# FKGSOFTWARE/TERRA-GAN

Measured on AMD Instinct MI355X. Metric: DSM tiles/sec train-step (G+D) at 256x256 bs=16, higher is better.
Workload: dtype f32; 1 GPU; BASELINE configs[1]: 256x256 1-ch DSM tiles, batch 16 per GPU, fp32, PConv-UNet G + PatchGAN D + L1/VGG-perceptual/TV/boundary(0.5) losses + 2x Adam; global_batch=16, tile=256, parallelism=single-gpu, launch=eager, vgg_weights=deterministic stand-in (ImageNet weights not fetchable offline; same FLOPs), vgg_trunk=forward Winograd F(2x2,3x3), dgrads F(4x4,3x3) (DESIGN 2b)

## Files before the change

### include/terragan_hip.h

```cpp
#ifndef TERRAGAN_HIP_H
#define TERRAGAN_HIP_H

#include <stddef.h>
#include <stdint.h>

#ifdef __cplusplus
extern "C" {
#endif

typedef void* tg_stream_t;

enum { TG_OK = 0, TG_ERR_ARG = -1, TG_ERR_LAUNCH = -2, TG_ERR_WS = -3 };
enum { TG_ACT_NONE = 0, TG_ACT_RELU = 1, TG_ACT_LEAKY = 2 };
enum { TG_PREC_F32 = 0, TG_PREC_BF16 = 1, TG_PREC_F32_WINO4 = 2 };

typedef struct TgConv {
    int32_t B, H, W, Cin;
    int32_t Ho, Wo, Cout;
    int32_t k, stride, pad;
    int32_t precision;
} TgConv;

int tg_version(void);
const char* tg_last_error(void);
// ... 20 lines not shown
int tg_conv_fwd_p(const TgConv* g, const float* x, const float* in_mask, const float* w, const float* wprep,
                  const float* bias, const float* ratio, int act, float slope, float* y, float* ws,
                  size_t ws_bytes, tg_stream_t stream);
int tg_conv_fwd_pool(const TgConv* g, const float* x, const float* in_mask, const float* w, const float* wprep,
                     const float* bias, const float* ratio, int act, float slope, float* y, float* pool_y, float* ws,
                     size_t ws_bytes, tg_stream_t stream);
int tg_conv_pool_code_supported(const TgConv* g);
int tg_conv_fwd_pool_code(const TgConv* g, const float* x, const float* w, const float* wprep, const float* bias,
                          float* pool_y, unsigned char* code, float* ws, size_t ws_bytes, tg_stream_t stream);
int tg_maxpool2_bwd_code(const float* dout, const unsigned char* code, int B, int Ho, int Wo, int C, float* dx,
                         tg_stream_t stream);
typedef struct TgSparseMap {
    const uint32_t* bits;
    const int32_t* list;
    const int32_t* count;
    const uint64_t* pix;
    int32_t nb, tiles_y, tiles_x, _pad;
} TgSparseMap;
size_t tg_vgg_sparse_map_bytes(int nb, int H, int W, const char* plan);
int tg_vgg_sparse_map(const float* x, const float* mask, int nb, int H, int W, const char* plan, void* buf, size_t buf_bytes,
                      int* ticket, TgSparseMap* maps, tg_stream_t stream);
int tg_conv_dgrad_sparse(const TgConv* g, const float* dy, const float* w, const float* wprep, const float* x_act, int act,
                         float slope, const uint32_t* gate_bits, float* dx, const TgSparseMap* sp, float* ws, size_t ws_bytes,
                         tg_stream_t stream);
int tg_conv_dgrad_sparse_planned(const TgConv* g, int gate, const TgSparseMap* sp);
int tg_maxpool2_bwd_code_sparse(const float* dout, const unsigned char* code, int B, int Ho, int Wo, int C, float* dx,
                                const TgSparseMap* sp, tg_stream_t stream);
int tg_conv_fwd_sparse(const TgConv* g, const float* x, const float* w, const float* wprep, const float* bias, int act,
                       float slope, float* y, float* pool_y, unsigned char* code, const TgSparseMap* sp, float* ws,
                       size_t ws_bytes, tg_stream_t stream);
typedef struct TgBnAct {
    const float *mean, *rstd, *gamma, *beta;
    int32_t act;
    float slope;
} TgBnAct;
int tg_conv_bnin_supported(const TgConv* g, int wgrad);
int tg_conv_fwd_bnin(const TgConv* g, const float* x, const TgBnAct* bn, const float* w, const float* bias, int act,
                     float slope, float* y, float* ws, size_t ws_bytes, tg_stream_t stream);
int tg_conv_wgrad_bnin(const TgConv* g, const float* x, const TgBnAct* bn, const float* dy, float* dw, float* db, float* ws,
                       size_t ws_bytes, tg_stream_t stream);
int tg_conv_dgrad_p(const TgConv* g, const float* dy, const float* w, const float* wprep, const float* in_mask,
                    const float* x_act, int act, float slope, float* dx, int accumulate, float* ws,
                    size_t ws_bytes, tg_stream_t stream);
int tg_relu_gate_pack(const float* a, int64_t rows, int C, uint32_t* bits, tg_stream_t stream);
int tg_conv_dgrad_gbits(const TgConv* g, const float* dy, const float* w, const float* wprep, const float* in_mask,
                        const uint32_t* gate_bits, float* dx, int accumulate, float* ws, size_t ws_bytes, tg_stream_t stream);

int tg_set_cu_reserve(int cus);
int tg_set_work_stealing(int mode);

size_t tg_conv_wgrad_ws_bytes(const TgConv* g);
int tg_conv_wgrad(const TgConv* g, const float* x, const float* in_mask, const float* dy,
                  float* dw, float* db, float* ws, size_t ws_bytes, tg_stream_t stream);

int tg_fold_cin(const float* w3, int cout, int taps, int cin, float* w1, tg_stream_t stream);


int tg_mask_update(const float* mask, int B, int H, int W, int k, int stride, int pad, int Ho,
                   int Wo, float* mask_out, float* ratio, tg_stream_t stream);
int tg_mask_up_merge(const float* up_mask, const float* skip_mask, int B, int h, int w, int H,
                     int W, float* out, tg_stream_t stream);

#define TG_MASK_PYRAMID_MAX 24
typedef struct TgMaskOp {
    int kind, H, W, Ho, Wo, k, stride, pad;
    const float* in;
    const float* in2;
    float* out;
    float* out2;
} TgMaskOp;
typedef struct TgMaskPyramid {
    int nops, _pad;
    TgMaskOp op[TG_MASK_PYRAMID_MAX];
} TgMaskPyramid;
int tg_mask_pyramid(const TgMaskPyramid* pm, int B, tg_stream_t stream);


size_t tg_bn_ws_bytes(int64_t rows, int C);
int tg_bn_stats(const float* y, int64_t rows, int C, float eps, float momentum, float* save_mean,
                float* save_rstd, float* running_mean, float* running_var,
                int64_t* num_batches_tracked, float* ws, size_t ws_bytes, tg_stream_t stream);
int tg_bn_fwd(const float* y, int64_t rows, int C, float eps, float momentum, const float* gamma,
              const float* beta, int act, float slope, float* save_mean, float* save_rstd,
              float* running_mean, float* running_var, int64_t* num_batches_tracked, float* out,
              float* ws, size_t ws_bytes, tg_stream_t stream);
int tg_bn_eval_stats(const float* running_mean, const float* running_var, int C, float eps,
                     float* mean, float* rstd, tg_stream_t stream);
int tg_bn_act_fwd(const float* y, int64_t rows, int C, const float* mean, const float* rstd,
                  const float* gamma, const float* beta, int act, float slope, float* out,
                  tg_stream_t stream);
int tg_bn_act_bwd(const float* dout, const float* y, int64_t rows, int C, const float* mean,
                  const float* rstd, const float* gamma, const float* beta, int act, float slope,
                  const float* ratio, float* dy, float* dgamma, float* dbeta, float* dbias, float* ws,
                  size_t ws_bytes, tg_stream_t stream);
int tg_bn_bwd_conv1_supported(int64_t rows, int C);
size_t tg_bn_conv1_ws_bytes(int64_t rows, int C);
int tg_bn_act_bwd_conv1(const float* dz, const float* w, int B, int H, int W, const float* y, int C, const float* mean,
                        const float* rstd, const float* gamma, const float* beta, int act, float slope, const float* ratio,
                        float* dy, float* dgamma, float* dbeta, float* dbias, float* ws, size_t ws_bytes, tg_stream_t stream);
int tg_act_bwd(const float* dout, const float* out, int64_t rows, int C, int act, float slope,
               const float* ratio, float* din, tg_stream_t stream);


int tg_upcat_fwd(const float* up, const float* skip, const float* out_mask, int B, int h, int w,
                 int Cu, int H, int W, int Cs, float* out, tg_stream_t stream);
int tg_upcat_bn_supported(int B, int h, int w, int Cu, int H, int W, int Cs);
// ... 308 lines not shown
```

### terra-gan_amd/csrc/pointwise.hip

```cpp
#include <math.h>
#include <string.h>

#include "common.h"

static thread_local char g_err[512] = "";
void tg_set_error(const char* fmt, ...) {
    va_list ap;
    va_start(ap, fmt);
    vsnprintf(g_err, sizeof(g_err), fmt, ap);
    va_end(ap);
}
extern "C" const char* tg_last_error(void) { return g_err; }
extern "C" int tg_version(void) { return 100; }

static size_t align_up(size_t v, size_t a) { return (v + a - 1) / a * a; }
static inline hipStream_t S(tg_stream_t s) { return (hipStream_t)s; }

constexpr int CR_MAXPASS = 4;

struct ColGeom {
    int cpp;
    int rlanes;
    int npass;
    int grid;
// ... 300 lines not shown
    TG_REQUIRE(pm && B > 0 && pm->nops >= 1 && pm->nops <= TG_MASK_PYRAMID_MAX, "tg_mask_pyramid: bad arguments");
    for (int i = 0; i < pm->nops; ++i) {
        const TgMaskOp& op = pm->op[i];
        TG_REQUIRE(op.in && op.out && (op.kind == 0 ? op.out2 != nullptr : op.in2 != nullptr), "tg_mask_pyramid: op %d: null pointer", i);
        TG_REQUIRE(op.H > 0 && op.W > 0 && op.Ho > 0 && op.Wo > 0, "tg_mask_pyramid: op %d: bad dims", i);
        if (op.kind == 0)
            TG_REQUIRE(op.k > 0 && op.stride > 0 && op.pad >= 0 && op.Ho == (op.H + 2 * op.pad - op.k) / op.stride + 1 &&
                       op.Wo == (op.W + 2 * op.pad - op.k) / op.stride + 1, "tg_mask_pyramid: op %d: Ho/Wo inconsistent", i);
    }
    hipLaunchKernelGGL(mask_pyramid_kernel, dim3(B), dim3(1024), 0, S(stream), *pm);
    TG_CHECK_LAUNCH("mask_pyramid_kernel");
    return TG_OK;
}

constexpr int VSM_MAX_OPS = 24, VSM_MAX_CONV = 16, VSM_LDS_WORDS = 4096;
struct VggMapArgs {
    const uint32_t* x;
    const float* mask;
    int nb, H, W, nops, nconv;
    char ops[VSM_MAX_OPS];
    int tiles_y[VSM_MAX_CONV], tiles_x[VSM_MAX_CONV];
    int32_t* count[VSM_MAX_CONV];
    uint32_t* bits[VSM_MAX_CONV];
    int32_t* list[VSM_MAX_CONV];
    unsigned char* flags[VSM_MAX_CONV];
    uint64_t* d0;
    int rows_per_slice;
    int* ticket;
};
__device__ __forceinline__ uint32_t vsm_even_bits(uint64_t v) {
    v &= 0x5555555555555555ull;
    v = (v | (v >> 1)) & 0x3333333333333333ull;
    v = (v | (v >> 2)) & 0x0f0f0f0f0f0f0f0full;
    v = (v | (v >> 4)) & 0x00ff00ff00ff00ffull;
    v = (v | (v >> 8)) & 0x0000ffff0000ffffull;
    v = (v | (v >> 16)) & 0x00000000ffffffffull;
    return (uint32_t)v;
}
__device__ __forceinline__ uint64_t vsm_row_mask(int W, int w, int WW) {
    return (w == WW - 1 && (W & 63)) ? (1ull << (W & 63)) - 1 : ~0ull;
}
__device__ __forceinline__ bool vsm_last_arrival(int* ctr, int n, int* s_last) {
    __builtin_amdgcn_s_waitcnt(0);
    __syncthreads();
    if (threadIdx.x == 0) {
        __threadfence();
        const bool last = atomicAdd(ctr, 1) == n - 1;
        if (last) __threadfence();
        *s_last = last;
    }
    __syncthreads();
    return *s_last;
}
__global__ __launch_bounds__(1024) void vgg_sparse_map_kernel(const VggMapArgs a) {
    extern __shared__ uint64_t vsm[];
    __shared__ int scan[1024];
    __shared__ int s_last;
    const int tid = threadIdx.x, lane = tid & 63, wave = tid >> 6, b = blockIdx.y;
    int H = a.H, W = a.W, WW = (W + 63) >> 6;
    uint64_t* cur = vsm;
    uint64_t* nxt = vsm + H * WW;
    uint64_t* d0 = a.d0 + (size_t)b * H * WW;
    {
        const uint32_t* xp = a.x + (size_t)b * H * W;
        const uint32_t* tp = a.x + ((size_t)a.nb + b) * H * W;
        const float* mp = a.mask ? a.mask + (size_t)b * H * W : nullptr;
        const int ubeg = blockIdx.x * a.rows_per_slice * WW, uend = min(H, (blockIdx.x + 1) * a.rows_per_slice) * WW;
        for (int u0 = ubeg + wave; u0 < uend; u0 += 16 * 8) {
            uint32_t pv[8], tv[8];
            float mv[8];
#pragma unroll
            for (int k = 0; k < 8; ++k) {
                const int u = u0 + 16 * k, y = u / WW, px = (u - y * WW) * 64 + lane;
                pv[k] = tv[k] = 0;
                mv[k] = 1.f;
                if (u < uend && px < W) {
                    pv[k] = xp[(size_t)y * W + px]; tv[k] = tp[(size_t)y * W + px];
                    if (mp) mv[k] = mp[(size_t)y * W + px];
                }
            }
#pragma unroll
            for (int k = 0; k < 8; ++k) {
                const uint64_t m = __ballot(pv[k] != tv[k] || mv[k] != 1.f);
                if (lane == 0 && u0 + 16 * k < uend) d0[u0 + 16 * k] = m;
            }
        }
    }
    if (!vsm_last_arrival(a.ticket + b, (int)gridDim.x, &s_last)) return;
    for (int u = tid; u < H * WW; u += 1024) cur[u] = d0[u];
    if (tid == 0) __hip_atomic_store(a.ticket + b, 0, __ATOMIC_RELAXED, __HIP_MEMORY_SCOPE_AGENT);
    __syncthreads();
    int ci = 0;
    for (int o = 0; o < a.nops; ++o) {
        if (a.ops[o] == 'C') {
            for (int u = tid; u < H * WW; u += 1024) {
                const int y = u / WW, w = u - y * WW;
                uint64_t r = 0;
                for (int dy = -1; dy <= 1; ++dy) {
                    const int yy = y + dy;
                    if (yy < 0 || yy >= H) continue;
                    const uint64_t* row = cur + yy * WW;
                    const uint64_t v = row[w];
                    r |= v | (v << 1) | (v >> 1);
                    if (w > 0) r |= row[w - 1] >> 63;
                    if (w + 1 < WW) r |= row[w + 1] << 63;
                }
                nxt[u] = r & vsm_row_mask(W, w, WW);
            }
            __syncthreads();
            uint64_t* t = cur; cur = nxt; nxt = t;
            const int ty_n = a.tiles_y[ci], tx_n = a.tiles_x[ci], tiles = ty_n * tx_n;
            for (int t2 = tid; t2 < tiles; t2 += 1024) {
                const int ty = t2 / tx_n, tx = t2 - ty * tx_n;
                const int w = (16 * tx) >> 6, sh = (16 * tx) & 63;
                uint64_t any = 0;
                for (int y = 16 * ty; y < min(16 * ty + 16, H); ++y) any |= (cur[y * WW + w] >> sh) & 0xffffull;
                a.flags[ci][(size_t)b * tiles + t2] = any ? 1 : 0;
            }
            ++ci;
        } else {
            const int H2 = H >> 1, W2 = W >> 1, WW2 = (W2 + 63) >> 6;
            for (int u = tid; u < H2 * WW2; u += 1024) {
                const int y = u / WW2, w = u - y * WW2;
                const uint64_t* r0 = cur + (2 * y) * WW;
                const uint64_t* r1 = r0 + WW;
                const uint64_t s0 = r0[2 * w] | r1[2 * w];
                const uint64_t s1 = 2 * w + 1 < WW ? r0[2 * w + 1] | r1[2 * w + 1] : 0;
                const uint64_t v = (uint64_t)vsm_even_bits(s0 | (s0 >> 1)) | ((uint64_t)vsm_even_bits(s1 | (s1 >> 1)) << 32);
                nxt[u] = v & vsm_row_mask(W2, w, WW2);
            }
            H = H2; W = W2; WW = WW2;
            __syncthreads();
            uint64_t* t = cur; cur = nxt; nxt = t;
        }
        __syncthreads();
    }
    if (!vsm_last_arrival(a.ticket + a.nb, a.nb, &s_last)) return;
    for (int c = 0; c < a.nconv; ++c) {
        const int n = a.nb * a.tiles_y[c] * a.tiles_x[c], nw = (n + 31) >> 5;
        int carry = 0;
        for (int w0 = 0; w0 < nw; w0 += 1024) {
            const int w = w0 + tid;
            uint32_t word = 0;
            if (w < nw) {
                const uint4* fp = reinterpret_cast<const uint4*>(a.flags[c] + 32 * (size_t)w);
                const uint4 f0 = fp[0], f1 = fp[1];
                const uint32_t fw[8] = {f0.x, f0.y, f0.z, f0.w, f1.x, f1.y, f1.z, f1.w};
#pragma unroll
                for (int i = 0; i < 8; ++i)
#pragma unroll
                    for (int j = 0; j < 4; ++j) word |= ((fw[i] >> (8 * j)) & 1u) << (4 * i + j);
                if (32 * w + 32 > n) word &= (1u << (n - 32 * w)) - 1u;
                a.bits[c][w] = word;
            }
            const int pc = __popc(word);
            scan[tid] = pc;
            __syncthreads();
            for (int d = 1; d < 1024; d <<= 1) {
                const int v = tid >= d ? scan[tid - d] : 0;
                __syncthreads();
                scan[tid] += v;
                __syncthreads();
            }
            int pos = carry + scan[tid] - pc;
            for (uint32_t m = word; m; m &= m - 1) a.list[c][pos++] = 32 * w + __ffs(m) - 1;
            carry += scan[1023];
            __syncthreads();
        }
        if (tid == 0) *a.count[c] = carry;
    }
    if (tid == 0) __hip_atomic_store(a.ticket + a.nb, 0, __ATOMIC_RELAXED, __HIP_MEMORY_SCOPE_AGENT);
}

struct VsmLayout {
    int nconv, nops, H, W;
    size_t d0;
    int tiles_y[VSM_MAX_CONV], tiles_x[VSM_MAX_CONV];
    size_t count[VSM_MAX_CONV], bits[VSM_MAX_CONV], list[VSM_MAX_CONV], flags[VSM_MAX_CONV];
    size_t bytes;
};
static bool vsm_layout(int nb, int H, int W, const char* plan, VsmLayout& L) {
    if (nb <= 0 || H <= 0 || W <= 0 || !plan) return false;
    if ((size_t)H * ((W + 63) / 64) > VSM_LDS_WORDS) return false;
    L = VsmLayout{};
    L.H = H; L.W = W;
    L.d0 = 0;
    size_t off = align_up((size_t)nb * H * ((W + 63) / 64) * sizeof(uint64_t), 16);
    int h = H, w = W;
    for (const char* c = plan; *c; ++c) {
        if (L.nops == VSM_MAX_OPS) return false;
        ++L.nops;
        if (*c == 'M') {
            h >>= 1; w >>= 1;
            if (h <= 0 || w <= 0) return false;
        } else if (*c == 'C') {
            if (L.nconv == VSM_MAX_CONV) return false;
            const int i = L.nconv++;
            L.tiles_y[i] = cdiv(h, 16); L.tiles_x[i] = cdiv(w, 16);
            const size_t n = (size_t)nb * L.tiles_y[i] * L.tiles_x[i];
            if (n > ((size_t)1 << 30)) return false;
            L.count[i] = off; off += 16;
            L.bits[i] = off; off += align_up((n + 31) / 32, 4) * 4;
            L.list[i] = off; off += align_up(n, 4) * 4;
            L.flags[i] = off; off += align_up(n, 32);
        } else {
            return false;
        }
    }
    L.bytes = off;
    return L.nconv > 0;
}
extern "C" size_t tg_vgg_sparse_map_bytes(int nb, int H, int W, const char* plan) {
    VsmLayout L;
    return vsm_layout(nb, H, W, plan, L) ? L.bytes : 0;
}
extern "C" int tg_vgg_sparse_map(const float* x, const float* mask, int nb, int H, int W, const char* plan, void* buf, size_t buf_bytes,
                                 int* ticket, TgSparseMap* maps, tg_stream_t stream) {
    VsmLayout L;
    TG_REQUIRE(x && buf && ticket && maps, "tg_vgg_sparse_map: null pointer");
    TG_REQUIRE(vsm_layout(nb, H, W, plan, L), "tg_vgg_sparse_map: geometry not supported (tg_vgg_sparse_map_bytes is 0)");
    TG_REQUIRE(buf_bytes >= L.bytes && (reinterpret_cast<uintptr_t>(buf) & 15) == 0, "tg_vgg_sparse_map: buffer too small or unaligned");
    VggMapArgs a = {};
    a.x = reinterpret_cast<const uint32_t*>(x);
    a.mask = mask;
    a.nb = nb; a.H = H; a.W = W; a.nops = L.nops; a.nconv = L.nconv; a.ticket = ticket;
    for (int i = 0; i < L.nops; ++i) a.ops[i] = plan[i];
    char* base = static_cast<char*>(buf);
    a.d0 = reinterpret_cast<uint64_t*>(base + L.d0);
    const int slices = cdiv(H, 8) < cdiv(256, nb) ? cdiv(H, 8) : cdiv(256, nb);
    a.rows_per_slice = cdiv(H, slices);
    for (int i = 0; i < L.nconv; ++i) {
        a.tiles_y[i] = L.tiles_y[i]; a.tiles_x[i] = L.tiles_x[i];
        a.count[i] = reinterpret_cast<int32_t*>(base + L.count[i]);
        a.bits[i] = reinterpret_cast<uint32_t*>(base + L.bits[i]);
        a.list[i] = reinterpret_cast<int32_t*>(base + L.list[i]);
        a.flags[i] = reinterpret_cast<unsigned char*>(base + L.flags[i]);
        maps[i] = TgSparseMap{a.bits[i], a.list[i], a.count[i], mask ? a.d0 : nullptr, nb, L.tiles_y[i], L.tiles_x[i], 0};
    }
    const size_t lds = 2 * (size_t)H * ((W + 63) / 64) * sizeof(uint64_t);
    static bool opted[64] = {};
    int dev = 0;
    (void)hipGetDevice(&dev);
    if (dev < 0 || dev >= 64 || !opted[dev]) {
        if (hipFuncSetAttribute(reinterpret_cast<const void*>(vgg_sparse_map_kernel), hipFuncAttributeMaxDynamicSharedMemorySize,
                                (int)(2 * VSM_LDS_WORDS * sizeof(uint64_t))) != hipSuccess) {
            tg_set_error("tg_vgg_sparse_map: LDS opt-in failed");
            return TG_ERR_LAUNCH;
        }
        if (dev >= 0 && dev < 64) opted[dev] = true;
    }
    hipLaunchKernelGGL(vgg_sparse_map_kernel, dim3(cdiv(H, a.rows_per_slice), nb), dim3(1024), lds, S(stream), a);
    TG_CHECK_LAUNCH("vgg_sparse_map_kernel");
    return TG_OK;
}

struct BnStatF {
    const float* y;
    int C;
    __device__ BnStatF group(int g, int64_t rows_g) const { return BnStatF{y + (size_t)g * rows_g * C, C}; }
    __device__ void operator()(int64_t r, int c, float (&q)[2]) const {
        float d = y[r * C + c] - y[c];
        q[0] += d;
        q[1] += d * d;
    }
    __device__ void quad(int64_t r, int c0, float (&q)[2][4]) const {
        const f32x4 v = *reinterpret_cast<const f32x4*>(y + r * C + c0);
        const f32x4 sh = *reinterpret_cast<const f32x4*>(y + c0);
#pragma unroll
        for (int e = 0; e < 4; ++e) {
            float d = v[e] - sh[e];
            q[0][e] += d;
            q[1][e] += d * d;
        }
    }
};
__global__ __launch_bounds__(256) void bn_finalize_kernel(const float* __restrict__ partial, int nblocks, int C,
                                                          const float* __restrict__ y, int64_t rows, float eps,
                                                          float momentum, float* __restrict__ mean_out,
                                                          float* __restrict__ rstd_out, float* __restrict__ rm,
                                                          float* __restrict__ rv, int64_t* __restrict__ nbt) {
    if (blockIdx.x == 0 && threadIdx.x == 0 && nbt) *nbt += 1;
    double q[2];
    int c;
    if (!final_reduce<2>(partial, nblocks, C, q, &c)) return;
    const double n = (double)rows;
    const double md = q[0] / n;
    double var = q[1] / n - md * md;
    if (var < 0.0) var = 0.0;
    const double mean = (double)y[c] + md;
    mean_out[c] = (float)mean;
    rstd_out[c] = (float)(1.0 / sqrt(var + (double)eps));
    if (rm) rm[c] = (float)((1.0 - (double)momentum) * (double)rm[c] + (double)momentum * mean);
    if (rv) rv[c] = (float)((1.0 - (double)momentum) * (double)rv[c] + (double)momentum * var * (n / (n - 1.0)));
}
extern "C" size_t tg_bn_ws_bytes(int64_t rows, int C) {
    if (rows <= 0 || C <= 0) return 0;
    ColGeom g = col_geom(rows, C);
    int grid = g.grid;
    if (C % 4 == 0) {
        ColGeom4 g4 = col_geom4(rows, C);
        if (g4.grid > grid) grid = g4.grid;
    }
    return align_up((size_t)grid * 5 * C, 64) * sizeof(float);
}
// ... 1858 lines not shown
```

### terra-gan_amd/csrc/wino.inc

```
#pragma once
#include <utility>

struct WinoGeom {
    int tiles_x, tiles_y, total_work, chunks_per_split, nt;
    int sy_min, sx_min;
    int interleave;
    int* qctr;
    const uint32_t* sp_bits;
    const int* sp_list;
    const int* sp_count;
    int sp_tiles, sp_nb;
};
struct WinoWeights {
    long sn, sk, stap;
    int kyu[3], kxv[3];
    int k_fast;
};
typedef unsigned int u32x4 __attribute__((ext_vector_type(4)));
constexpr int WINO_BN = 64;
constexpr int WINO_V = 16 * 64 * 8;
constexpr int WINO_U = 16 * WINO_BN * 8;
constexpr int WINO_PPIX = 18 * 18;
constexpr int WINO_P = WINO_PPIX * 8;
constexpr int WINO_LDS_FLOATS = 2 * WINO_V + 2 * WINO_U + WINO_P;
// ... 1074 lines not shown
#pragma unroll
    for (int i = 0; i < 8; ++i)
#pragma unroll
        for (int r = 0; r < 16; ++r) {
            const int row = 32 * mw + (r & 3) + 8 * (r >> 2) + 4 * (lane >> 5);
            slab[(size_t)i * 4096 + row * 64 + 32 * nw + (lane & 31)] = acc[i][r];
        }
}

__global__ __launch_bounds__(256) void wino_wgrad_reduce_kernel(const float* __restrict__ slabs, float* __restrict__ dw, int Cout,
                                                                int Cin, int ntco, int ntci, int splits) {
    const int total = Cout * Cin;
    for (int idx = blockIdx.x * 256 + threadIdx.x; idx < total; idx += gridDim.x * 256) {
        const int col = idx & 63, row = (idx >> 6) & 63, tile = idx >> 12;
        const int tco = tile % ntco, tci = tile / ntco;
        float u[16];
#pragma unroll
        for (int i = 0; i < 16; ++i) u[i] = 0.f;
        const size_t sstride = (size_t)ntci * ntco * 16 * 4096;
        const float* sl = slabs + ((size_t)tile * 16) * 4096 + row * 64 + col;
        int sp = 0;
        for (; sp + 4 <= splits; sp += 4) {
            float v[4][16];
#pragma unroll
            for (int k = 0; k < 4; ++k)
#pragma unroll
                for (int i = 0; i < 16; ++i) v[k][i] = sl[(size_t)(sp + k) * sstride + (size_t)i * 4096];
#pragma unroll
            for (int k = 0; k < 4; ++k)
#pragma unroll
                for (int i = 0; i < 16; ++i) u[i] += v[k][i];
        }
        for (; sp < splits; ++sp)
#pragma unroll
            for (int i = 0; i < 16; ++i) u[i] += sl[(size_t)sp * sstride + (size_t)i * 4096];
        float t[3][4];
#pragma unroll
        for (int b = 0; b < 4; ++b) {
            t[0][b] = u[0 * 4 + b] + 0.5f * (u[1 * 4 + b] + u[2 * 4 + b]);
            t[1][b] = 0.5f * (u[1 * 4 + b] - u[2 * 4 + b]);
            t[2][b] = 0.5f * (u[1 * 4 + b] + u[2 * 4 + b]) + u[3 * 4 + b];
        }
        const int co = tco * 64 + 4 * (row & 15) + (row >> 4), ci = tci * 64 + 4 * (col & 15) + (col >> 4);
        float* o = dw + ((size_t)co * 9) * Cin + ci;
#pragma unroll
        for (int uu = 0; uu < 3; ++uu) {
            o[(size_t)(uu * 3 + 0) * Cin] = t[uu][0] + 0.5f * (t[uu][1] + t[uu][2]);
            o[(size_t)(uu * 3 + 1) * Cin] = 0.5f * (t[uu][1] - t[uu][2]);
            o[(size_t)(uu * 3 + 2) * Cin] = 0.5f * (t[uu][1] + t[uu][2]) + t[uu][3];
        }
    }
}

static bool wino_wgrad_ok(const TgConv* g, const float* in_mask) {
    static const bool off = getenv("TG_NO_WINO") != nullptr || getenv("TG_NO_WINO_WGRAD") != nullptr;
    if (off || in_mask != nullptr) return false;
    if (g->precision == TG_PREC_BF16 && g->Cin > 256) return false;
    if (g->k != 3 || g->stride != 1 || (g->Cin % 64) != 0 || (g->Cout % 64) != 0 || g->Ho < 16 || g->Wo < 16) return false;
    if ((size_t)g->B * g->H * g->W * g->Cin * 4 >= ((size_t)1 << 31) || (size_t)g->B * g->Ho * g->Wo * g->Cout * 4 >= ((size_t)1 << 31))
        return false;
    return true;
}
static WinoWgradGeom wino_wgrad_plan(const TgConv* g) {
    WinoWgradGeom q = {};
    q.strips_x = cdiv(g->Wo, 16);
    q.tiles_y = cdiv(g->Ho, 2);
    q.nstrips = g->B * q.tiles_y * q.strips_x;
    q.ntco = g->Cout / 64;
    q.ntci = g->Cin / 64;
    const int tiles = q.ntco * q.ntci;
    int smax = q.nstrips / 8 < 512 ? q.nstrips / 8 : 512;
    if (smax < 1) smax = 1;
    const int splits = choose_splits_k(tiles, smax, WINO_PLAN_CUS, q.nstrips, 0.03);
    q.steps_per_split = cdiv(q.nstrips, splits);
    q.splits = cdiv(q.nstrips, q.steps_per_split);
    return q;
}
static size_t wino_wgrad_ws_floats(const TgConv* g) {
    if (!wino_wgrad_ok(g, nullptr)) return 0;
    const WinoWgradGeom q = wino_wgrad_plan(g);
    return (size_t)q.splits * q.ntco * q.ntci * 16 * 4096;
}
static int launch_wino_wgrad(const TgConv* g, const WgradParams& p, float* dw, float* ws, hipStream_t s) {
    const WinoWgradGeom q = wino_wgrad_plan(g);
    const size_t lds = (size_t)WINO_WG_LDS_FLOATS * sizeof(float);
    static LdsOptIn opt;
    if (int rc = lds_opt_in(opt, reinterpret_cast<const void*>(wino_wgrad_kernel), lds, "wino wgrad")) return rc;
    {
        const double by = 4.0 * ((double)p.B * p.H * p.W * p.C + (double)p.Mpix * p.Cout + (double)p.Cout * p.Ktot);
        ProfScope ps(s, 1, 2.0 * p.Mpix * (double)p.Cout * p.Ktot * g_alg_scale, by, p.Cout, p.Ktot, p.Mpix, p.C, q.splits, 4164);
        ps.r.route = WR_WGRAD;
        hipLaunchKernelGGL(wino_wgrad_kernel, dim3(q.ntco * q.ntci * q.splits), dim3(WINO_THREADS), lds, s, p, q, ws);
    }
    TG_CHECK_LAUNCH("wino_wgrad_kernel");
    hipLaunchKernelGGL(wino_wgrad_reduce_kernel, dim3(ew_grid((int64_t)g->Cout * g->Cin, 256)), dim3(256), 0, s, ws, dw, g->Cout,
                       g->Cin, q.ntco, q.ntci, q.splits);
    TG_CHECK_LAUNCH("wino_wgrad_reduce_kernel");
    return TG_OK;
}
```

### terra-gan_amd/csrc/wino16.inc

```
#pragma once

constexpr int W16_IMG = 16 * 64 * 16;
constexpr int W16_P = WINO_PPIX * 16;
constexpr size_t W16_LDS_BYTES = 4 * (size_t)W16_IMG * 2 + (size_t)W16_P * 4;
constexpr int W16_PP = WINO_PPIX * 24;
constexpr size_t W16_PIPE_LDS_BYTES = 4 * (size_t)W16_IMG * 2 + (size_t)W16_PP * 4;

__host__ __device__ __forceinline__ int w16_pos(int row, int c) { return ((((c >> 3) ^ (row >> 4)) & 1) << 3) + (c & 7); }

__device__ void wino_weights16_body(const float* __restrict__ w, __bf16* __restrict__ U, int N, int K, const WinoWeights& ww) {
    const int NT = N / WINO_BN, K2 = K >> 1;
    const size_t total = (size_t)N * K2;
    for (size_t idx = (size_t)blockIdx.x * 256 + threadIdx.x; idx < total; idx += (size_t)gridDim.x * 256) {
        int n, k2;
        if (ww.k_fast) { k2 = (int)(idx % K2); n = (int)(idx / K2); }
        else { n = (int)(idx % N); k2 = (int)(idx / N); }
        float u[2][16];
#pragma unroll
        for (int h = 0; h < 2; ++h) {
            const float* wp = w + (size_t)n * ww.sn + (size_t)(2 * k2 + h) * ww.sk;
            float g[3][3];
#pragma unroll
            for (int a = 0; a < 3; ++a)
#pragma unroll
// ... 709 lines not shown
            }
        }
    }
    float* slab = slabs + ((size_t)work * 16 + 8 * xh) * 4096;
#pragma unroll
    for (int i = 0; i < 8; ++i)
#pragma unroll
        for (int r = 0; r < 16; ++r) {
            const int row = 32 * mw + (r & 3) + 8 * (r >> 2) + 4 * (lane >> 5);
            slab[(size_t)i * 4096 + row * 64 + 32 * nw + (lane & 31)] = acc[i][r];
        }
}

static bool wino16_wgrad_ok(const TgConv* g, const float* in_mask) {
    static const bool off = getenv("TG_NO_WINO") != nullptr || getenv("TG_NO_WINO_WGRAD") != nullptr || getenv("TG_NO_WINO16") != nullptr ||
                            getenv("TG_NO_WINO16_WGRAD") != nullptr;
    if (off || in_mask != nullptr || g->precision != TG_PREC_BF16) return false;
    if (g->k != 3 || g->stride != 1 || (g->Cin % 64) != 0 || (g->Cout % 64) != 0 || g->Ho < 16 || g->Wo < 32) return false;
    if ((size_t)g->B * g->H * g->W * g->Cin * 4 >= ((size_t)1 << 31) || (size_t)g->B * g->Ho * g->Wo * g->Cout * 4 >= ((size_t)1 << 31))
        return false;
    return true;
}
static WinoWgradGeom wino16_wgrad_plan(const TgConv* g) {
    WinoWgradGeom q = {};
    q.strips_x = cdiv(g->Wo, 32);
    q.tiles_y = cdiv(g->Ho, 2);
    q.nstrips = g->B * q.tiles_y * q.strips_x;
    q.ntco = g->Cout / 64;
    q.ntci = g->Cin / 64;
    const int tiles = q.ntco * q.ntci;
    int smax = q.nstrips / 4 < 512 ? q.nstrips / 4 : 512;
    if (smax < 1) smax = 1;
    const int splits = choose_splits_k(tiles, smax, WINO_PLAN_CUS, q.nstrips, 0.03);
    q.steps_per_split = cdiv(q.nstrips, splits);
    q.splits = cdiv(q.nstrips, q.steps_per_split);
    return q;
}
static size_t wino16_wgrad_ws_floats(const TgConv* g) {
    if (!wino16_wgrad_ok(g, nullptr)) return 0;
    const WinoWgradGeom q = wino16_wgrad_plan(g);
    return (size_t)q.splits * q.ntco * q.ntci * 16 * 4096;
}
static int launch_wino16_wgrad(const TgConv* g, const WgradParams& p, float* dw, float* ws, hipStream_t s) {
    const WinoWgradGeom q = wino16_wgrad_plan(g);
    static LdsOptIn opt;
    if (int rc = lds_opt_in(opt, reinterpret_cast<const void*>(wino16_wgrad_kernel), W16G_LDS_BYTES, "wino16 wgrad")) return rc;
    {
        const double by = 4.0 * ((double)p.B * p.H * p.W * p.C + (double)p.Mpix * p.Cout + (double)p.Cout * p.Ktot);
        ProfScope ps(s, 3, 2.0 * p.Mpix * (double)p.Cout * p.Ktot * g_alg_scale, by, p.Cout, p.Ktot, p.Mpix, p.C, q.splits, 4116);
        ps.r.route = WR_WGRAD;
        hipLaunchKernelGGL(wino16_wgrad_kernel, dim3(q.ntco * q.ntci * q.splits), dim3(WINO_THREADS), W16G_LDS_BYTES, s, p, q, ws);
    }
    TG_CHECK_LAUNCH("wino16_wgrad_kernel");
    hipLaunchKernelGGL(wino_wgrad_reduce_kernel, dim3(ew_grid((int64_t)g->Cout * g->Cin, 256)), dim3(256), 0, s, ws, dw, g->Cout,
                       g->Cin, q.ntco, q.ntci, q.splits);
    TG_CHECK_LAUNCH("wino_wgrad_reduce_kernel");
    return TG_OK;
}
```

### terra-gan_amd/tg_hip/lib.py

```python
import ctypes as C
import os

import torch

_HERE = os.path.dirname(os.path.abspath(__file__))
LIB_PATH = os.environ.get("TG_HIP_LIB") or os.path.join(os.path.dirname(_HERE), "lib", "libterragan_hip.so")


class TgConv(C.Structure):
    _fields_ = [(n, C.c_int32) for n in ("B", "H", "W", "Cin", "Ho", "Wo", "Cout", "k", "stride", "pad", "precision")]


TG_MASK_PYRAMID_MAX = 24


class TgMaskOp(C.Structure):
    _fields_ = [(n, C.c_int32) for n in ("kind", "H", "W", "Ho", "Wo", "k", "stride", "pad")] + \
               [(n, C.c_void_p) for n in ("in_", "in2", "out", "out2")]


class TgMaskPyramid(C.Structure):
    _fields_ = [("nops", C.c_int32), ("_pad", C.c_int32), ("op", TgMaskOp * TG_MASK_PYRAMID_MAX)]


# ... 7 lines not shown

class TgRasterPlan(C.Structure):
    _fields_ = [(n, C.c_int32) for n in ("H", "W", "wh", "ww", "overlap", "ny", "nx")]


TG_EVAL_MAX_CLASSES = 8


class TgAreaClasses(C.Structure):
    _fields_ = [("n_edges", C.c_int32), ("_pad", C.c_int32), ("px", C.c_int64 * (TG_EVAL_MAX_CLASSES - 1))]


TG_EDT_FAR, TG_EDT_MAX_SIDE, TG_DEPTH_MAX_CLASSES = 0x7fffffff, 32767, 8


class TgDepthClasses(C.Structure):
    _fields_ = [("n_edges", C.c_int32), ("_pad", C.c_int32), ("d2", C.c_int32 * (TG_DEPTH_MAX_CLASSES - 1))]


TG_FLOW_OUT, TG_FLOW_UNDECIDED, TG_FLOW_PIT, TG_FLOW_FAR, TG_FLOW_MAX_ROUNDS = 9, 254, 255, 0x7fffffff, 32
TG_FLOW_BASIN_COUNTS, TG_FLOW_COMPARE_COUNTS = 3, 19
TG_STREAM_HEAD, TG_STREAM_INTERIOR, TG_STREAM_JUNCTION, TG_STREAM_ORDER_BINS = 1, 2, 3, 15
TG_STREAM_ORDER_COUNTS = 1 + 2 * TG_STREAM_ORDER_BINS
TG_FLOOD_MAX_STAGES = 8
TG_FLOOD_COUNTS = 6 + 3 * TG_FLOOD_MAX_STAGES
TG_MFD_MAX_EXPONENT, TG_MFD_COUNTS = 8, 5
TG_TEX_OCTAVES, TG_TEX_SCALES, TG_TEX_NSUM = 5, 10, 3
TG_VGM_OCTAVES, TG_VGM_SCALES = 6, 12
TG_VGM_POWER, TG_VGM_EXPONENTIAL, TG_VGM_SPHERICAL = 0, 1, 2


class TgFloodStages(C.Structure):
    _fields_ = [("s", C.c_float * TG_FLOOD_MAX_STAGES)]


class TgError(RuntimeError):
    pass


P, I, I64, F, SZ, D = C.c_void_p, C.c_int, C.c_int64, C.c_float, C.c_size_t, C.c_double
CP = C.POINTER(TgConv)
RP = C.POINTER(TgRasterPlan)

SIGNATURES = {
    "tg_version": (I, []),
    "tg_last_error": (C.c_char_p, []),
    "tg_conv_fwd_ws_bytes": (SZ, [CP]),
    "tg_conv_fwd": (I, [CP, P, P, P, P, P, I, F, P, P, SZ, P]),
    "tg_conv_dgrad_ws_bytes": (SZ, [CP]),
    "tg_conv_dgrad": (I, [CP, P, P, P, P, I, P, SZ, P]),
    "tg_conv_dgrad_gated": (I, [CP, P, P, P, P, I, F, P, P, SZ, P]),
    "tg_set_cu_reserve": (I, [I]),
    "tg_set_work_stealing": (I, [I]),
    "tg_conv_wprep_bytes": (SZ, [CP, I]),
    "tg_conv_wprep": (I, [CP, I, P, P, P]),
    "tg_conv_wprep_item_bytes": (SZ, []),
    "tg_conv_wprep_item": (I, [CP, I, P, P, P]),
    "tg_conv_wprep_run": (I, [P, I, P]),
    "tg_conv_fwd_p": (I, [CP, P, P, P, P, P, P, I, F, P, P, SZ, P]),
    "tg_conv_fwd_pool": (I, [CP, P, P, P, P, P, P, I, F, P, P, P, SZ, P]),
    "tg_conv_pool_code_supported": (I, [CP]),
    "tg_conv_fwd_pool_code": (I, [CP, P, P, P, P, P, P, P, SZ, P]),
    "tg_maxpool2_bwd_code": (I, [P, P, I, I, I, I, P, P]),
    "tg_vgg_sparse_map_bytes": (SZ, [I, I, I, C.c_char_p]),
    "tg_vgg_sparse_map": (I, [P, P, I, I, I, C.c_char_p, P, SZ, P, C.POINTER(TgSparseMap), P]),
    "tg_conv_dgrad_sparse": (I, [CP, P, P, P, P, I, F, P, P, C.POINTER(TgSparseMap), P, SZ, P]),
    "tg_conv_dgrad_sparse_planned": (I, [CP, I, C.POINTER(TgSparseMap)]),
    "tg_maxpool2_bwd_code_sparse": (I, [P, P, I, I, I, I, P, C.POINTER(TgSparseMap), P]),
    "tg_conv_fwd_sparse": (I, [CP, P, P, P, P, I, F, P, P, P, C.POINTER(TgSparseMap), P, SZ, P]),
    "tg_conv_bnin_supported": (I, [CP, I]),
    "tg_conv_fwd_bnin": (I, [CP, P, C.POINTER(TgBnAct), P, P, I, F, P, P, SZ, P]),
    "tg_conv_wgrad_bnin": (I, [CP, P, C.POINTER(TgBnAct), P, P, P, P, SZ, P]),
    "tg_conv_dgrad_p": (I, [CP, P, P, P, P, P, I, F, P, I, P, SZ, P]),
    "tg_relu_gate_pack": (I, [P, I64, I, P, P]),
    "tg_conv_dgrad_gbits": (I, [CP, P, P, P, P, P, P, I, P, SZ, P]),
    "tg_conv_wgrad_ws_bytes": (SZ, [CP]),
    "tg_conv_wgrad": (I, [CP, P, P, P, P, P, P, SZ, P]),
    "tg_fold_cin": (I, [P, I, I, I, P, P]),
    "tg_mask_update": (I, [P, I, I, I, I, I, I, I, I, P, P, P]),
    "tg_mask_up_merge": (I, [P, P, I, I, I, I, I, P, P]),
    "tg_mask_pyramid": (I, [C.POINTER(TgMaskPyramid), I, P]),
    "tg_bn_ws_bytes": (SZ, [I64, I]),
    "tg_bn_stats": (I, [P, I64, I, F, F, P, P, P, P, P, P, SZ, P]),
    "tg_bn_eval_stats": (I, [P, P, I, F, P, P, P]),
    "tg_bn_act_fwd": (I, [P, I64, I, P, P, P, P, I, F, P, P]),
    "tg_bn_fwd": (I, [P, I64, I, F, F, P, P, I, F, P, P, P, P, P, P, P, SZ, P]),
    "tg_bn_act_bwd": (I, [P, P, I64, I, P, P, P, P, I, F, P, P, P, P, P, P, SZ, P]),
    "tg_bn_bwd_conv1_supported": (I, [I64, I]),
    "tg_bn_conv1_ws_bytes": (SZ, [I64, I]),
    "tg_bn_act_bwd_conv1": (I, [P, P, I, I, I, P, I, P, P, P, P, I, F, P, P, P, P, P, P, SZ, P]),
    "tg_act_bwd": (I, [P, P, I64, I, I, F, P, P, P]),
    "tg_upcat_fwd": (I, [P, P, P, I, I, I, I, I, I, I, P, P]),
    "tg_upcat_bn_supported": (I, [I, I, I, I, I, I, I]),
    "tg_upcat_fwd_bn": (I, [P, C.POINTER(TgBnAct), P, P, I, I, I, I, I, I, I, P, P]),
    "tg_upcat_bwd": (I, [P, I, I, I, I, I, I, I, P, P, P]),
    "tg_sigmoid_composite_fwd": (I, [P, P, P, I64, P, P]),
    "tg_sigmoid_composite_bwd": (I, [P, P, P, I64, P, P, P]),
    "tg_maxpool2_fwd": (I, [P, I, I, I, I, P, P]),
    "tg_maxpool2_bwd": (I, [P, P, I, I, I, I, I, P, P]),
    "tg_pixel_loss_ws_bytes": (SZ, [I, I, I]),
    "tg_pixel_losses": (I, [P, P, P, P, I, I, I, F, F, F, F, P, P, P, I, P, SZ, P]),
    "tg_reduce_ws_bytes": (SZ, [I64]),
    "tg_l1_mean": (I, [P, P, I64, F, P, P, P, P, SZ, P]),
    "tg_l1_mean_relu": (I, [P, P, I64, F, P, P, P, P, SZ, P]),
    "tg_bce_logits": (I, [P, I64, F, F, P, P, P, P, SZ, P]),
    "tg_adam": (I, [P, P, P, P, I64, D, D, D, D, I, F, P]),
# ... 125 lines not shown
```

Measured before the change: 1088 tiles/s.

## Split VGG sparse-map kernel into staged launches and widen Winograd wgrad reduce

```diff
diff --git a/include/terragan_hip.h b/include/terragan_hip.h
--- a/include/terragan_hip.h
+++ b/include/terragan_hip.h
@@ -96,6 +96,7 @@
 size_t tg_conv_wgrad_ws_bytes(const TgConv* g);
 int tg_conv_wgrad(const TgConv* g, const float* x, const float* in_mask, const float* dy,
                   float* dw, float* db, float* ws, size_t ws_bytes, tg_stream_t stream);
+int64_t tg_wgrad_reduce_wide_launches(void);
 
 int tg_fold_cin(const float* w3, int cout, int taps, int cin, float* w1, tg_stream_t stream);
 
diff --git a/terra-gan_amd/csrc/pointwise.hip b/terra-gan_amd/csrc/pointwise.hip
--- a/terra-gan_amd/csrc/pointwise.hip
+++ b/terra-gan_amd/csrc/pointwise.hip
@@ -376,6 +376,7 @@
     __syncthreads();
     return *s_last;
 }
+template <int STAGE>
 __global__ __launch_bounds__(1024) void vgg_sparse_map_kernel(const VggMapArgs a) {
     extern __shared__ uint64_t vsm[];
     __shared__ int scan[1024];
@@ -385,7 +386,7 @@
     uint64_t* cur = vsm;
     uint64_t* nxt = vsm + H * WW;
     uint64_t* d0 = a.d0 + (size_t)b * H * WW;
-    {
+    if constexpr (STAGE == 0 || STAGE == 1) {
         const uint32_t* xp = a.x + (size_t)b * H * W;
         const uint32_t* tp = a.x + ((size_t)a.nb + b) * H * W;
         const float* mp = a.mask ? a.mask + (size_t)b * H * W : nullptr;
@@ -410,57 +411,64 @@
             }
         }
     }
-    if (!vsm_last_arrival(a.ticket + b, (int)gridDim.x, &s_last)) return;
-    for (int u = tid; u < H * WW; u += 1024) cur[u] = d0[u];
-    if (tid == 0) __hip_atomic_store(a.ticket + b, 0, __ATOMIC_RELAXED, __HIP_MEMORY_SCOPE_AGENT);
-    __syncthreads();
-    int ci = 0;
-    for (int o = 0; o < a.nops; ++o) {
-        if (a.ops[o] == 'C') {
-            for (int u = tid; u < H * WW; u += 1024) {
-                const int y = u / WW, w = u - y * WW;
-                uint64_t r = 0;
-                for (int dy = -1; dy <= 1; ++dy) {
-                    const int yy = y + dy;
-                    if (yy < 0 || yy >= H) continue;
-                    const uint64_t* row = cur + yy * WW;
-                    const uint64_t v = row[w];
-                    r |= v | (v << 1) | (v >> 1);
-                    if (w > 0) r |= row[w - 1] >> 63;
-                    if (w + 1 < WW) r |= row[w + 1] << 63;
+    if constexpr (STAGE == 1) return;
+    if constexpr (STAGE == 0)
+        if (!vsm_last_arrival(a.ticket + b, (int)gridDim.x, &s_last)) return;
+    if constexpr (STAGE == 0 || STAGE == 2) {
+        for (int u = tid; u < H * WW; u += 1024) cur[u] = d0[u];
+        if constexpr (STAGE == 0)
+            if (tid == 0) __hip_atomic_store(a.ticket + b, 0, __ATOMIC_RELAXED, __HIP_MEMORY_SCOPE_AGENT);
+        __syncthreads();
+        int ci = 0;
+        for (int o = 0; o < a.nops; ++o) {
+            if (a.ops[o] == 'C') {
+                for (int u = tid; u < H * WW; u += 1024) {
+                    const int y = u / WW, w = u - y * WW;
+                    uint64_t r = 0;
+                    for (int dy = -1; dy <= 1; ++dy) {
+                        const int yy = y + dy;
+                        if (yy < 0 || yy >= H) continue;
+                        const uint64_t* row = cur + yy * WW;
+                        const uint64_t v = row[w];
+                        r |= v | (v << 1) | (v >> 1);
+                        if (w > 0) r |= row[w - 1] >> 63;
+                        if (w + 1 < WW) r |= row[w + 1] << 63;
+                    }
+                    nxt[u] = r & vsm_row_mask(W, w, WW);
                 }
-                nxt[u] = r & vsm_row_mask(W, w, WW);
+                __syncthreads();
+                uint64_t* t = cur; cur = nxt; nxt = t;
+                const int ty_n = a.tiles_y[ci], tx_n = a.tiles_x[ci], tiles = ty_n * tx_n;
+                for (int t2 = tid; t2 < tiles; t2 += 1024) {
+                    const int ty = t2 / tx_n, tx = t2 - ty * tx_n;
+                    const int w = (16 * tx) >> 6, sh = (16 * tx) & 63;
+                    uint64_t any = 0;
+                    for (int y = 16 * ty; y < min(16 * ty + 16, H); ++y) any |= (cur[y * WW + w] >> sh) & 0xffffull;
+                    a.flags[ci][(size_t)b * tiles + t2] = any ? 1 : 0;
+                }
+                ++ci;
+            } else {
+                const int H2 = H >> 1, W2 = W >> 1, WW2 = (W2 + 63) >> 6;
+                for (int u = tid; u < H2 * WW2; u += 1024) {
+                    const int y = u / WW2, w = u - y * WW2;
+                    const uint64_t* r0 = cur + (2 * y) * WW;
+                    const uint64_t* r1 = r0 + WW;
+                    const uint64_t s0 = r0[2 * w] | r1[2 * w];
+                    const uint64_t s1 = 2 * w + 1 < WW ? r0[2 * w + 1] | r1[2 * w + 1] : 0;
+                    const uint64_t v = (uint64_t)vsm_even_bits(s0 | (s0 >> 1)) | ((uint64_t)vsm_even_bits(s1 | (s1 >> 1)) << 32);
+                    nxt[u] = v & vsm_row_mask(W2, w, WW2);
+                }
+                H = H2; W = W2; WW = WW2;
+                __syncthreads();
+                uint64_t* t = cur; cur = nxt; nxt = t;
             }
             __syncthreads();
-            uint64_t* t = cur; cur = nxt; nxt = t;
-            const int ty_n = a.tiles_y[ci], tx_n = a.tiles_x[ci], tiles = ty_n * tx_n;
-            for (int t2 = tid; t2 < tiles; t2 += 1024) {
-                const int ty = t2 / tx_n, tx = t2 - ty * tx_n;
-                const int w = (16 * tx) >> 6, sh = (16 * tx) & 63;
-                uint64_t any = 0;
-                for (int y = 16 * ty; y < min(16 * ty + 16, H); ++y) any |= (cur[y * WW + w] >> sh) & 0xffffull;
-                a.flags[ci][(size_t)b * tiles + t2] = any ? 1 : 0;
-            }
-            ++ci;
-        } else {
-            const int H2 = H >> 1, W2 = W >> 1, WW2 = (W2 + 63) >> 6;
-            for (int u = tid; u < H2 * WW2; u += 1024) {
-                const int y = u / WW2, w = u - y * WW2;
-                const uint64_t* r0 = cur + (2 * y) * WW;
-                const uint64_t* r1 = r0 + WW;
-                const uint64_t s0 = r0[2 * w] | r1[2 * w];
-                const uint64_t s1 = 2 * w + 1 < WW ? r0[2 * w + 1] | r1[2 * w + 1] : 0;
-                const uint64_t v = (uint64_t)vsm_even_bits(s0 | (s0 >> 1)) | ((uint64_t)vsm_even_bits(s1 | (s1 >> 1)) << 32);
-                nxt[u] = v & vsm_row_mask(W2, w, WW2);
-            }
-            H = H2; W = W2; WW = WW2;
-            __syncthreads();
-            uint64_t* t = cur; cur = nxt; nxt = t;
-        }
-        __syncthreads();
-    }
-    if (!vsm_last_arrival(a.ticket + a.nb, a.nb, &s_last)) return;
-    for (int c = 0; c < a.nconv; ++c) {
+        }
+    }
+    if constexpr (STAGE == 2) return;
+    if constexpr (STAGE == 0)
+        if (!vsm_last_arrival(a.ticket + a.nb, a.nb, &s_last)) return;
+    for (int c = STAGE == 3 ? (int)blockIdx.x : 0; c < (STAGE == 3 ? (int)blockIdx.x + 1 : a.nconv); ++c) {
         const int n = a.nb * a.tiles_y[c] * a.tiles_x[c], nw = (n + 31) >> 5;
         int carry = 0;
         for (int w0 = 0; w0 < nw; w0 += 1024) {
@@ -493,7 +501,12 @@
         }
         if (tid == 0) *a.count[c] = carry;
     }
-    if (tid == 0) __hip_atomic_store(a.ticket + a.nb, 0, __ATOMIC_RELAXED, __HIP_MEMORY_SCOPE_AGENT);
+    if constexpr (STAGE == 0)
+        if (tid == 0) __hip_atomic_store(a.ticket + a.nb, 0, __ATOMIC_RELAXED, __HIP_MEMORY_SCOPE_AGENT);
+}
+static bool vsm_split_enabled() {
+    const char* e = getenv("TG_VGG_MAP_SPLIT");
+    return e == nullptr || atoi(e) != 0;
 }
 
 struct VsmLayout {
@@ -566,14 +579,25 @@
     int dev = 0;
     (void)hipGetDevice(&dev);
     if (dev < 0 || dev >= 64 || !opted[dev]) {
-        if (hipFuncSetAttribute(reinterpret_cast<const void*>(vgg_sparse_map_kernel), hipFuncAttributeMaxDynamicSharedMemorySize,
-                                (int)(2 * VSM_LDS_WORDS * sizeof(uint64_t))) != hipSuccess) {
-            tg_set_error("tg_vgg_sparse_map: LDS opt-in failed");
-            return TG_ERR_LAUNCH;
-        }
+        const void* staged[2] = {reinterpret_cast<const void*>(vgg_sparse_map_kernel<0>), reinterpret_cast<const void*>(vgg_sparse_map_kernel<2>)};
+        for (const void* k : staged)
+            if (hipFuncSetAttribute(k, hipFuncAttributeMaxDynamicSharedMemorySize, (int)(2 * VSM_LDS_WORDS * sizeof(uint64_t))) !=
+                hipSuccess) {
+                tg_set_error("tg_vgg_sparse_map: LDS opt-in failed");
+                return TG_ERR_LAUNCH;
+            }
         if (dev >= 0 && dev < 64) opted[dev] = true;
     }
-    hipLaunchKernelGGL(vgg_sparse_map_kernel, dim3(cdiv(H, a.rows_per_slice), nb), dim3(1024), lds, S(stream), a);
+    if (vsm_split_enabled()) {
+        hipLaunchKernelGGL(vgg_sparse_map_kernel<1>, dim3(cdiv(H, a.rows_per_slice), nb), dim3(1024), 0, S(stream), a);
+        TG_CHECK_LAUNCH("vgg_sparse_map_kernel<1>");
+        hipLaunchKernelGGL(vgg_sparse_map_kernel<2>, dim3(1, nb), dim3(1024), lds, S(stream), a);
+        TG_CHECK_LAUNCH("vgg_sparse_map_kernel<2>");
+        hipLaunchKernelGGL(vgg_sparse_map_kernel<3>, dim3(a.nconv, 1), dim3(1024), 0, S(stream), a);
+        TG_CHECK_LAUNCH("vgg_sparse_map_kernel<3>");
+        return TG_OK;
+    }
+    hipLaunchKernelGGL(vgg_sparse_map_kernel<0>, dim3(cdiv(H, a.rows_per_slice), nb), dim3(1024), lds, S(stream), a);
     TG_CHECK_LAUNCH("vgg_sparse_map_kernel");
     return TG_OK;
 }
diff --git a/terra-gan_amd/csrc/wino.inc b/terra-gan_amd/csrc/wino.inc
--- a/terra-gan_amd/csrc/wino.inc
+++ b/terra-gan_amd/csrc/wino.inc
@@ -1150,6 +1150,111 @@
     }
 }
 
+constexpr int WGR_RING = 32;
+__global__ __launch_bounds__(256) void wino_wgrad_reduce_wide_kernel(const float* __restrict__ slabs, float* __restrict__ dw, int Cout,
+                                                                     int Cin, int ntco, int ntci, int splits) {
+    __shared__ float su[16][16];
+    const int e = threadIdx.x & 15, pt = threadIdx.x >> 4;
+    const int idx = xcd_remap(blockIdx.x, gridDim.x) * 16 + e;
+    const int col = idx & 63, row = (idx >> 6) & 63, tile = idx >> 12;
+    const int tco = tile % ntco, tci = tile / ntco;
+    const size_t sstride = (size_t)ntci * ntco * 16 * 4096;
+    const int last = splits - 1;
+    const float* q = slabs + ((size_t)tile * 16 + pt) * 4096 + row * 64 + col;
+    float v[WGR_RING];
+    float acc = 0.f;
+    int done = 0;
+    if (2 * WGR_RING < splits) {
+#pragma unroll
+        for (int k = 0; k < WGR_RING; ++k) {
+            v[k] = *q;
+            q += sstride;
+        }
+        for (; done + 2 * WGR_RING < splits; done += WGR_RING) {
+#pragma unroll
+            for (int k = 0; k < WGR_RING; ++k) {
+                acc += v[k];
+                v[k] = *q;
+                q += sstride;
+                __builtin_amdgcn_sched_barrier(0);
+            }
+        }
+    } else {
+#pragma unroll
+        for (int g = 0; g < WGR_RING; g += 8) {
+#pragma unroll
+            for (int k = g; k < g + 8; ++k) v[k] = 0.f;
+            if (g < splits) {
+#pragma unroll
+                for (int k = g; k < g + 8; ++k) {
+                    v[k] = *q;
+                    q += k < last ? sstride : 0;
+                }
+            }
+        }
+    }
+#pragma nounroll
+    for (; done < splits; done += WGR_RING) {
+#pragma unroll
+        for (int g = 0; g < WGR_RING; g += 8) {
+            float x[8];
+#pragma unroll
+            for (int k = 0; k < 8; ++k) x[k] = v[g + k];
+            if (done + WGR_RING + g < splits) {
+#pragma unroll
+                for (int k = g; k < g + 8; ++k) {
+                    v[k] = *q;
+                    q += done + WGR_RING + k < last ? sstride : 0;
+                }
+            }
+#pragma unroll
+            for (int k = 0; k < 8; ++k) acc = done + g + k < splits ? acc + x[k] : acc;
+        }
+    }
+    su[pt][e] = acc;
+    __syncthreads();
+    if (pt != 0) return;
+    float u[16];
+#pragma unroll
+    for (int i = 0; i < 16; ++i) u[i] = su[i][e];
+    float t[3][4];
+#pragma unroll
+    for (int b = 0; b < 4; ++b) {
+        t[0][b] = u[0 * 4 + b] + 0.5f * (u[1 * 4 + b] + u[2 * 4 + b]);
+        t[1][b] = 0.5f * (u[1 * 4 + b] - u[2 * 4 + b]);
+        t[2][b] = 0.5f * (u[1 * 4 + b] + u[2 * 4 + b]) + u[3 * 4 + b];
+    }
+    const int co = tco * 64 + 4 * (row & 15) + (row >> 4), ci = tci * 64 + 4 * (col & 15) + (col >> 4);
+    float* o = dw + ((size_t)co * 9) * Cin + ci;
+#pragma unroll
+    for (int uu = 0; uu < 3; ++uu) {
+        o[(size_t)(uu * 3 + 0) * Cin] = t[uu][0] + 0.5f * (t[uu][1] + t[uu][2]);
+        o[(size_t)(uu * 3 + 1) * Cin] = 0.5f * (t[uu][1] - t[uu][2]);
+        o[(size_t)(uu * 3 + 2) * Cin] = 0.5f * (t[uu][1] + t[uu][2]) + t[uu][3];
+    }
+}
+
+static std::atomic<long long> g_wgrad_reduce_wide_launches{0};
+extern "C" int64_t tg_wgrad_reduce_wide_launches(void) { return (int64_t)g_wgrad_reduce_wide_launches.load(std::memory_order_relaxed); }
+static bool wino_wgrad_reduce_wide(const TgConv* g) {
+    const char* e = getenv("TG_WGRAD_REDUCE_WIDE");
+    if (e != nullptr && atoi(e) == 0) return false;
+    return 4 * ew_grid((int64_t)g->Cout * g->Cin, 256) <= WINO_PLAN_CUS;
+}
+static int launch_wino_wgrad_reduce(const TgConv* g, const WinoWgradGeom& q, const float* ws, float* dw, hipStream_t s) {
+    if (wino_wgrad_reduce_wide(g)) {
+        hipLaunchKernelGGL(wino_wgrad_reduce_wide_kernel, dim3(g->Cout * g->Cin / 16), dim3(256), 0, s, ws, dw, g->Cout, g->Cin, q.ntco,
+                           q.ntci, q.splits);
+        TG_CHECK_LAUNCH("wino_wgrad_reduce_wide_kernel");
+        g_wgrad_reduce_wide_launches.fetch_add(1, std::memory_order_relaxed);
+        return TG_OK;
+    }
+    hipLaunchKernelGGL(wino_wgrad_reduce_kernel, dim3(ew_grid((int64_t)g->Cout * g->Cin, 256)), dim3(256), 0, s, ws, dw, g->Cout, g->Cin,
+                       q.ntco, q.ntci, q.splits);
+    TG_CHECK_LAUNCH("wino_wgrad_reduce_kernel");
+    return TG_OK;
+}
+
 static bool wino_wgrad_ok(const TgConv* g, const float* in_mask) {
     static const bool off = getenv("TG_NO_WINO") != nullptr || getenv("TG_NO_WINO_WGRAD") != nullptr;
     if (off || in_mask != nullptr) return false;
@@ -1191,8 +1296,5 @@
         hipLaunchKernelGGL(wino_wgrad_kernel, dim3(q.ntco * q.ntci * q.splits), dim3(WINO_THREADS), lds, s, p, q, ws);
     }
     TG_CHECK_LAUNCH("wino_wgrad_kernel");
-    hipLaunchKernelGGL(wino_wgrad_reduce_kernel, dim3(ew_grid((int64_t)g->Cout * g->Cin, 256)), dim3(256), 0, s, ws, dw, g->Cout,
-                       g->Cin, q.ntco, q.ntci, q.splits);
-    TG_CHECK_LAUNCH("wino_wgrad_reduce_kernel");
-    return TG_OK;
-}
+    return launch_wino_wgrad_reduce(g, q, ws, dw, s);
+}
diff --git a/terra-gan_amd/csrc/wino16.inc b/terra-gan_amd/csrc/wino16.inc
--- a/terra-gan_amd/csrc/wino16.inc
+++ b/terra-gan_amd/csrc/wino16.inc
@@ -785,8 +785,5 @@
         hipLaunchKernelGGL(wino16_wgrad_kernel, dim3(q.ntco * q.ntci * q.splits), dim3(WINO_THREADS), W16G_LDS_BYTES, s, p, q, ws);
     }
     TG_CHECK_LAUNCH("wino16_wgrad_kernel");
-    hipLaunchKernelGGL(wino_wgrad_reduce_kernel, dim3(ew_grid((int64_t)g->Cout * g->Cin, 256)), dim3(256), 0, s, ws, dw, g->Cout,
-                       g->Cin, q.ntco, q.ntci, q.splits);
-    TG_CHECK_LAUNCH("wino_wgrad_reduce_kernel");
-    return TG_OK;
-}
+    return launch_wino_wgrad_reduce(g, q, ws, dw, s);
+}
diff --git a/terra-gan_amd/tg_hip/lib.py b/terra-gan_amd/tg_hip/lib.py
--- a/terra-gan_amd/tg_hip/lib.py
+++ b/terra-gan_amd/tg_hip/lib.py
@@ -83,6 +83,7 @@
     "tg_conv_dgrad_gated": (I, [CP, P, P, P, P, I, F, P, P, SZ, P]),
     "tg_set_cu_reserve": (I, [I]),
     "tg_set_work_stealing": (I, [I]),
+    "tg_wgrad_reduce_wide_launches": (I64, []),
     "tg_conv_wprep_bytes": (SZ, [CP, I]),
     "tg_conv_wprep": (I, [CP, I, P, P, P]),
     "tg_conv_wprep_item_bytes": (SZ, []),
```

After: 1092 tiles/s, median of 6. No clear change (+0.3%).
